# qradiolink/qradiolink

Hardware: AMD Instinct MI355X
Metric: IQ MSamples/sec through RX demod chain (higher is better)
Workload: dtype f32

## Files before the change

### qradiolink_amd/csrc/demod.hpp

```cpp
#pragma once
#include "host_common.hpp"
#include "firdes.hpp"
#include <utility>

namespace qrl {

inline std::vector<float> decim_layout(const std::vector<float>& h, int D, int Jpad)
{
    std::vector<float> t((size_t)D * Jpad, 0.0f);
    for (size_t k = 0; k < h.size(); ++k) t[(k % D) * Jpad + k / D] = h[k];
    return t;
}
inline std::vector<float> resamp_layout(const std::vector<float>& h, int I, int Jp)
{
    std::vector<float> t((size_t)I * Jp, 0.0f);
    for (size_t k = 0; k < h.size(); ++k) t[(k % I) * Jp + k / I] = h[k];
    return t;
}
inline std::vector<float2> to_f2(const std::vector<std::complex<float>>& v)
{
    std::vector<float2> r(v.size());
    for (size_t i = 0; i < v.size(); ++i) r[i] = make_float2(v[i].real(), v[i].imag());
    return r;
}

struct DecimStage {
    bool used = false;
    DecimChoice c{DECIM_CLASS_GENERIC, DECIM_R4_J12, 0};
    int D = 1, nt = 0, S = 0;
    DevBuf<float> taps;
    DevBuf<float2> edge, edge_b; uint32_t edge_len = 0;
    int alloc_edge(int B, bool two = false) {
        edge_len = (uint32_t)(c.cls == DECIM_CLASS_PM ? decim_pm_edge_len(nt, D) : c.cls == DECIM_CLASS_PL ? decim_pl_edge_len(nt, D) : 0);
        if (!edge_len) return QRL_OK;
        if (int r = edge.alloc((size_t)B * edge_len)) return r;
// ... 41 lines not shown
    DevBuf<float> f1, f2, f3; uint32_t m1 = 0, m2 = 0; DevBuf<AnState> st;
    float tone = 0.0f; DevBuf<CtcssState> cs; DevBuf<float> f4, ftaps_ct; DevBuf<double> env_ct; int nf_ct = 0;
    float wr[3] = {0, 0, 0}, wi[3] = {0, 0, 0};
    double threshold = 1e-14, ff[2] = {0, 0}, fb1 = 0, de_ff[2] = {0, 0}, de_fb1 = 0;
    float gain = 1.f, attack = 0.1f, decay = 0.1f, if_gain = 0.9f;
    int build(qrl_demod& d, size_t max2);
    int init_state(qrl_demod& d);
    int stages(qrl_demod& d, uint64_t n2_0, uint64_t n2_1, const qrl_demod_out* out, uint32_t* counts);
};

struct DsssChain {
    DevBuf<float> rs, filt, mf; int Jp = 0, nf = 0;
    DevBuf<float2> ra, rb, rc, rd, sym; uint32_t mask = 0, sym_mask = 0;
    DevBuf<DsssState> st; DevBuf<DsssTailState> tail;
    float a1 = 0, b1 = 0, a2 = 0, b2 = 0;
    uint64_t n5 = 0, nsy = 0;
    int build(qrl_demod& d, size_t max2);
    int init_state(qrl_demod& d);
    int stages(qrl_demod& d, uint64_t n2_0, uint64_t n2_1, const qrl_demod_out* out, uint32_t* counts);
};

}

using namespace qrl;

struct qrl_demod {
    qrl_ctx* ctx = nullptr;
    qrl_demod_config cfg{};
    hipStream_t stream = nullptr;
    bool own_stream = false;
    hipStream_t tail = nullptr;
    hipStream_t fecs = nullptr;
    hipEvent_t ev_q[2] = {nullptr, nullptr}, ev_fec[2] = {nullptr, nullptr}; bool q_valid[2] = {false, false};
    bool grouped = false, grouped_capable = false, fec_deferred = false; FecParams fec_pending{}; int fec_pending_slot = 0;
    DevBuf<uint64_t> qp_snap;
    hipEvent_t ev_ff = nullptr, ev_tail = nullptr;
    hipStream_t pre = nullptr; hipEvent_t ev_pre = nullptr, ev_fe[2] = {nullptr, nullptr}; bool fe_valid[2] = {false, false}; bool pre_pending = false;
    bool input_resident = false;
    hipEvent_t ev_user[4] = {nullptr, nullptr, nullptr, nullptr};
    bool tail_pending = false;
    bool qpsk_fll = false, fsk4_disc = false;
    bool m17 = false;
    DevBuf<float2> s2g, disc4_taps; DevBuf<float> sym4_taps; int disc4_nt = 0, sym4_nt = 0;
    bool fll_slim = false;
    bool d2f_capable = false, d2f = false; DevBuf<float> d2f_taps;
    bool overlap = false, overlap_capable = false; hipEvent_t ev_tail2[2] = {nullptr, nullptr}; bool tail2_valid[2] = {false, false}; uint64_t call_no = 0;
    enum Family { F_2FSK, F_GMSK, F_QPSK, F_DMR, F_4FSK, F_BPSK, F_DSSS, F_ANALOG } fam = F_2FSK;
    int branches = 2;

    int fe_decim = 1, interp = 1, decim = 1, target = 0, sps_eff = 0;
    bool fm = false;

    DecimStage fe;
    DecimStage first;
    DecimStage scope; DevBuf<float2> s_scope; uint32_t scope_mask = 0; uint64_t n_scope = 0; int scope_D = 10;
    float2* scope_out = nullptr; size_t scope_cap = 0; uint32_t* scope_counts = nullptr;
    DevBuf<float> rs_taps; int rs_Jp = 0;
    DevBuf<float> filt_taps; int filt_nt = 0;
    DevBuf<float> symf_taps; int symf_nt = 0;
    DevBuf<float2> disc_up, disc_lo; int disc_nt = 0;
    DevBuf<float> ff_tf, ff_ts; DevBuf<float2> ff_up, ff_lo;
    DevBuf<float2> fll_lo, fll_up; float fll_alpha = 0, fll_beta = 0, fll_maxf = 0;
    DevBuf<float> atan_tab, mmse_tab;
    float demod_gain = 0;
    float ss_alpha = 0, ss_beta = 0, ss_maxp = 0, ss_minp = 0;

    Rotator rot;

    DevBuf<float2> hist_a, hist_b; uint32_t hist_len = 0; bool hist_flip = false;
    DevBuf<float2> s1, s2, s2l, s2f; DevBuf<float> s2d, s3; DevBuf<uint8_t> soft;
    uint32_t s1_mask = 0, s2_mask = 0, soft_mask = 0;
    DevBuf<FllState> fll_st; DevBuf<SymSyncState> ss_st; DevBuf<FecState> fec_st;
    DevBuf<DmoState> dmo_st; DevBuf<uint32_t> dmo_golay; uint8_t* dmo_out = nullptr; uint32_t dmo_cap = 0; uint32_t* dmo_counts = nullptr;
    DevBuf<QpskState> qp_st; DevBuf<float> tanh_tab;
    float c1_alpha = 0, c1_beta = 0, c2_alpha = 0, c2_beta = 0; float2 qp_rot{};
    DevBuf<uint32_t> counts_scratch;
    AnalogChain an;
    DsssChain ds;
    uint64_t n_in = 0, n1 = 0, n2 = 0;
    bool profiling = false;
    std::vector<std::pair<hipEvent_t, hipEvent_t>> prof_events;

    ~qrl_demod() {
        for (auto& e : prof_events) { (void)hipEventDestroy(e.first); (void)hipEventDestroy(e.second); }
        if (ev_ff) (void)hipEventDestroy(ev_ff);
        if (ev_tail) (void)hipEventDestroy(ev_tail);
        for (auto e : ev_user) if (e) (void)hipEventDestroy(e);
        for (auto e : ev_tail2) if (e) (void)hipEventDestroy(e);
        for (auto e : ev_q) if (e) (void)hipEventDestroy(e);
        for (auto e : ev_fec) if (e) (void)hipEventDestroy(e);
        if (ev_pre) (void)hipEventDestroy(ev_pre);
        for (auto e : ev_fe) if (e) (void)hipEventDestroy(e);
        if (pre) (void)hipStreamDestroy(pre);
        if (fecs) (void)hipStreamDestroy(fecs);
        if (tail) (void)hipStreamDestroy(tail);
        if (own_stream && stream) (void)hipStreamDestroy(stream);
    }

    int flush_fec(bool behind_front_end);
    int sync_all() {
        if (int r = flush_fec(false)) return r;
        HIPCHK(hipStreamSynchronize(stream));
        HIPCHK(hipStreamSynchronize(tail));
        HIPCHK(hipStreamSynchronize(fecs));
        if (pre) HIPCHK(hipStreamSynchronize(pre));
        return QRL_OK;
    }
    bool loops_family() const { return fam == F_QPSK || fam == F_BPSK || fsk4_disc; }
    int init_state();
    int build();
    int process(const void* iq, size_t stride, size_t n, const qrl_demod_out* out, int fmt = IN_CF32);
    float sc16_scale = 1.0f / 32768.0f;
    int init_dmo_state() { DmoState x; std::memset(&x, 0, sizeof x); x.endPtr = 9999; return dmo_st.fill(cfg.batch, x); }
    CallCounts call_counts(size_t n) const {
        const size_t c1 = fe.used ? n / fe_decim + 2 : n, c2 = c1 * interp / decim + 2;
        return {c1, c2, c2 / (size_t)(sps_eff > 1 ? sps_eff - 1 : 1) + 8};
    }
    PortC filtered_port(const qrl_demod_out* out) const { return cfg.enable_side_outputs && out ? PortC{reinterpret_cast<float2*>(out->filtered), out->filtered_cap} : PortC{nullptr, 0}; }
    PortC constellation_port(const qrl_demod_out* out) const { return cfg.enable_side_outputs && out ? PortC{reinterpret_cast<float2*>(out->constellation), out->constellation_cap} : PortC{nullptr, 0}; }
    template <class P> void input_source(P& p, const float2* in, size_t stride, const float2* hist_old, uint64_t src0, uint64_t src1) const {
        if (fe.used) { p.in = nullptr; p.in_ring = RingC{s1.p, s1_mask}; }
        else { p.in = in; p.in_stride = stride; p.hist = hist_old; p.hist_len = hist_len; p.rot_enable = 1; rot.fill(p); }
        p.n0 = src0; p.n = (uint32_t)(src1 - src0);
// ... 3 lines not shown
```

### qradiolink_amd/csrc/engine.cpp

```cpp
#include "demod.hpp"
#include <cmath>
#include <cstdlib>
#include <memory>
#include <new>

#ifndef QRL_FEC_GATE_US
#define QRL_FEC_GATE_US 30u
#endif
#ifndef QRL_DEV_SKIP
#define QRL_DEV_SKIP 0
#endif

int qrl_demod::flush_fec(bool behind_front_end)
{
    if (!fec_deferred) return QRL_OK;
    fec_deferred = false;
    HIPCHK(hipStreamWaitEvent(fecs, ev_q[fec_pending_slot], 0));
    if (behind_front_end) {
        HIPCHK(hipStreamWaitEvent(fecs, ev_ff, 0));
        launch_fec_gate(QRL_FEC_GATE_US, fecs);
    }
    launch_fec(fec_pending, cfg.batch, fecs);
    HIPCHK(hipEventRecord(ev_fec[fec_pending_slot], fecs));
    return QRL_OK;
// ... 101 lines not shown
    const uint32_t first_look = interp == 1 ? std::max<uint32_t>(first.lookback(), d2f ? dec2_fir_lookback() : 0u) : 0u;
    {
        const int sr = cfg.time_domain_samp_rate;
        if (sr < 0 || sr > 500000 || cfg.time_domain_filter_width < 0 || cfg.time_domain_filter_width > 500000) return qrl_set_error(QRL_ERR_ARG, "time_domain_samp_rate / filter_width out of range");
        scope_D = sr > 0 ? 1000000 / sr : 10;
        if (sr > 0 && sr / 2 - sr / 8 <= 0) return qrl_set_error(QRL_ERR_ARG, "time_domain_samp_rate too small");
        const std::vector<float> h = cfg.time_domain_filter_width > 0 ? low_pass(1, 1000000, cfg.time_domain_filter_width, cfg.time_domain_filter_width, WIN_HAMMING)
                                   : sr > 0 ? low_pass(1, 1000000, sr / 2 - sr / 8, sr / 4, WIN_HAMMING)
                                            : low_pass(1, 1000000, 50000, 25000, WIN_HAMMING);
        if (h.size() > 4096) return qrl_set_error(QRL_ERR_ARG, "time-domain filter too long (> 4096 taps)");
        if ((r = scope.plan(h, scope_D))) return qrl_set_error(r, "scope plan");
    }
    if (!fe.used && (r = scope.alloc_edge(cfg.batch))) return qrl_set_error(r, "scope edge scratch");
    if (fe.used) hist_len = fe.lookback();
    else if (interp == 1) hist_len = std::max(first_look, scope.lookback());
    else hist_len = std::max((uint32_t)(rs_Jp + decim + 2), scope.lookback());
    if ((r = hist_a.alloc((size_t)B * hist_len)) || (r = hist_b.alloc((size_t)B * hist_len))) return r;

    const CallCounts mx = call_counts(cfg.max_chunk);
    if (fe.used) {
        const size_t look = std::max<size_t>(interp == 1 ? first_look : (size_t)(rs_Jp + decim + 2), scope.lookback());
        s1_mask = pow2_at_least(mx.n1 + look + 64, 64) - 1;
        if ((r = s1.alloc((size_t)B * (s1_mask + 1)))) return r;
    }
    overlap_capable = fam == F_2FSK;
    grouped_capable = fam == F_QPSK && !fsk4_disc;
    {
        int dev = 0, cus = 256; hipDeviceProp_t pr;
        if (hipGetDevice(&dev) == hipSuccess && hipGetDeviceProperties(&pr, dev) == hipSuccess) cus = pr.multiProcessorCount;
        grouped = grouped_capable && 2 * ((B + 63) / 64) >= cus;
    }
    overlap = overlap_capable;
    s2_mask = pow2_at_least((overlap_capable || loops_family() ? 2 : 1) * mx.n2 + (fam == F_DMR ? 2048 : fam == F_ANALOG ? 4096 : 1024), 64) - 1;
    const size_t ring2 = (size_t)B * (s2_mask + 1);
    if ((r = s2.alloc(ring2)) || (r = s2f.alloc(ring2)) || (r = s2d.alloc(ring2)) || (r = s3.alloc(ring2))) return r;
    if ((fam == F_2FSK || fam == F_BPSK || (fam == F_QPSK && qpsk_fll)) && (r = s2l.alloc(ring2))) return r;
    soft_mask = pow2_at_least((loops_family() ? 2 : 1) * (fam == F_QPSK || fam == F_4FSK ? 2 : 1) * mx.nsym + 512, 64) - 1;
    if ((r = soft.alloc((size_t)B * (soft_mask + 1)))) return r;

    {
        const std::vector<float> f = fam == F_QPSK
            ? root_raised_cosine(sps_eff, sps_eff, 1, 0.35, 11 * sps_eff)
            : fam == F_BPSK
            ? root_raised_cosine(sps_eff, sps_eff, 1, 0.35, 15 * sps_eff)
            : fam == F_4FSK
            ? low_pass(1, target, fw, fw / 2, WIN_BLACKMAN_HARRIS)
            : fam == F_ANALOG
            ? (an.kind == 2 ? low_pass_2(1, target, fw, 600, 90, WIN_BLACKMAN_HARRIS)
                            : low_pass_2(1, target, fw, 3500, 60, WIN_BLACKMAN_HARRIS))
            : low_pass(1, target, fw, fw, WIN_BLACKMAN_HARRIS);
        filt_nt = (int)f.size();
        if ((r = filt_taps.upload(f))) return r;
    }
    if ((r = atan_tab.upload(atan_table())) || (r = mmse_tab.upload(mmse_table()))) return r;
    if (fam == F_2FSK) {
        std::vector<std::complex<float>> lo, up;
        fll_band_edge_taps((float)sps_eff, 0.1f, 16, lo, up);
        if ((r = fll_lo.upload(to_f2(lo))) || (r = fll_up.upload(to_f2(up)))) return r;
        control_loop_gains((float)(24 * M_PI / 100), fll_alpha, fll_beta);
        fll_maxf = (float)(2 * M_PI * (2.0 / sps_eff));
        if ((r = fll_st.alloc(B))) return r;
        if (fm) {
            int nfilts = (sps == 1 ? 125 : 35) * sps_eff;
            if ((nfilts % 2) == 0) nfilts += 1;
            const std::vector<float> rrc = root_raised_cosine(1, target, target / sps_eff, 0.2, nfilts);
            symf_nt = (int)rrc.size();
// ... 83 lines not shown
            fll_maxf = (float)(2 * M_PI * (2.0 / sps_eff));
            if ((r = fll_st.alloc(B))) return r;
        }
        const float symbol_rate = (float)target / (float)sps_eff;
        const float dev = 200.0f / symbol_rate;
        clock_loop_gains((float)(2 * M_PI / (symbol_rate / 10)), 1.0f, 0.2869f, ss_alpha, ss_beta);
        ss_maxp = (float)sps_eff + dev; ss_minp = (float)sps_eff - dev;
        const float ang = (float)(-3 * M_PI / 4);
        qp_rot = make_float2((float)std::cos((double)ang), (float)std::sin((double)ang));
    } else {
        const std::vector<float> sf = low_pass(1, target, target / sps_eff, target / sps_eff, WIN_HAMMING);
        symf_nt = (int)sf.size();
        if ((r = symf_taps.upload(sf))) return r;
        demod_gain = (float)(sps_eff / (M_PI / 2));
        clock_loop_gains((float)(2 * M_PI / 200.0f), 1.0f, 0.2869f, ss_alpha, ss_beta);
        ss_maxp = (float)sps_eff + 0.05f; ss_minp = (float)sps_eff - 0.05f;
    }
    if ((r = ss_st.alloc(B)) || (r = fec_st.alloc((size_t)B * 2)) || (r = counts_scratch.alloc((size_t)B * 4))) return r;
    if (loops_family() && (r = qp_snap.alloc((size_t)B * 2))) return r;
    if ((fam == F_ANALOG && (r = an.build(*this, mx.n2))) || (fam == F_DSSS && (r = ds.build(*this, mx.n2)))) return r;
    return init_state();
}

int qrl_demod::process(const void* iq, size_t stride, size_t n, const qrl_demod_out* out, int fmt)
{
    if (fmt == IN_SC16 && !fe.used)
        return qrl_set_error(QRL_ERR_ARG, "qrl_demod_process_sc16: int16 input needs the device-rate front end (device_samp_rate >= 2000000); this handle runs at 1 Msps");
    if (n > cfg.max_chunk) return qrl_set_error(QRL_ERR_TOO_BIG, "n exceeds max_chunk");
    if (fmt == IN_SC16) {
        if (!sc16_rows_ok("qrl_demod_process_sc16", iq, stride)) return QRL_ERR_ARG;
    } else if ((reinterpret_cast<uintptr_t>(iq) & 15u) || (stride & 1u)) return qrl_set_error(QRL_ERR_ARG, "iq must be 16-byte aligned, stride even");
    const int B = cfg.batch;
    uint32_t* counts = (out && out->counts) ? out->counts : counts_scratch.p;
    hipStream_t cs = overlap ? tail : stream;
    const int slot = (int)(call_no & 1);
    if (overlap) {
        if (tail2_valid[slot]) HIPCHK(hipStreamWaitEvent(stream, ev_tail2[slot], 0));
    } else {
        HIPCHK(hipMemsetAsync(counts, 0, (size_t)B * 4 * sizeof(uint32_t), stream));
    }
    if (loops_family() && q_valid[slot]) HIPCHK(hipStreamWaitEvent(stream, ev_q[slot], 0));
    if (grouped && q_valid[slot ^ 1]) HIPCHK(hipStreamWaitEvent(stream, ev_q[slot ^ 1], 0));
    if (pre_pending) { HIPCHK(hipStreamWaitEvent(stream, ev_pre, 0)); pre_pending = false; }
    const bool use_pre = pre && input_resident;
    const float2* in = reinterpret_cast<const float2*>(iq);
    const float2* hist_old = hist_flip ? hist_b.p : hist_a.p;
    const PortC fport = filtered_port(out), cport = constellation_port(out);
    float2* hist_new = hist_flip ? hist_a.p : hist_b.p;

    const uint64_t n_in0 = n_in, n_in1 = n_in + n;
    uint64_t n1_0 = n1, n1_1 = n1;
    RingC r2{s2.p, s2_mask}, r2l{s2l.p, s2_mask}, r2f{s2f.p, s2_mask};
    RingF r2d{s2d.p, s2_mask}, r3{s3.p, s2_mask};

    hipEvent_t ev0 = nullptr, ev1 = nullptr;
    if (profiling) {
        HIPCHK(hipEventCreate(&ev0)); HIPCHK(hipEventCreate(&ev1));
        HIPCHK(hipEventRecord(ev0, stream));
    }
    if (fe.used) {
        n1_1 = decim_count(n_in1, 1, fe_decim);
        DecimParams p{};
        p.in = in; p.in_stride = stride; p.n0 = n_in0; p.n = (uint32_t)n;
        p.hist = hist_old; p.hist_len = hist_len;
        p.out = RingC{s1.p, s1_mask}; p.m0 = n1_0; p.m_count = (uint32_t)(n1_1 - n1_0);
        p.taps = fe.taps.p; p.D = fe.D; p.Jpad = fe.c.Jpad;
        p.rot_enable = 1; rot.fill(p);
        p.in_fmt = fmt; p.in_scale = sc16_scale;
        if (use_pre) { p.pre_stream = pre; p.pre_event = ev_pre; }
// ... 25 lines not shown
            p.port = fport.p; p.port_cap = fport.cap; p.port_counts = counts;
        }
        launch_resamp(p, B, stream);
    }
    if (profiling && !fe.used) { HIPCHK(hipEventRecord(ev1, stream)); prof_events.emplace_back(ev0, ev1); }
    if (scope_out) {
        const uint64_t ns_1 = decim_count(src1, 1, scope_D);
        DecimParams p{};
        input_source(p, in, stride, hist_old, src0, src1);
        p.out = RingC{s_scope.p, scope_mask}; p.m0 = n_scope; p.m_count = (uint32_t)(ns_1 - n_scope);
        p.taps = scope.taps.p; p.D = scope.D; p.Jpad = scope.c.Jpad;
        if (scope.launch(p, B, stream)) return qrl_set_error(QRL_ERR_HIP, "scope launch: hipFuncSetAttribute failed");
        launch_ring_store(RingC{s_scope.p, scope_mask}, n_scope, (uint32_t)(ns_1 - n_scope), scope_out, scope_cap, scope_counts, B, stream);
        n_scope = ns_1;
    }
    {
        HistParams h{};
        h.in = in; h.in_stride = stride; h.n0 = n_in0; h.n = (uint32_t)n;
        h.hist_old = hist_old; h.hist_new = hist_new; h.hist_len = hist_len;
        h.rot_enable = 1; rot.fill(h);
        h.in_fmt = fmt; h.in_scale = sc16_scale;
        if (pre) { HIPCHK(hipEventRecord(ev_fe[slot], stream)); fe_valid[slot] = true; }
        if (use_pre) {
            if (fe_valid[slot ^ 1]) HIPCHK(hipStreamWaitEvent(pre, ev_fe[slot ^ 1], 0));
            launch_hist_save(h, B, pre);
            HIPCHK(hipEventRecord(ev_pre, pre));
            pre_pending = true;
        } else launch_hist_save(h, B, stream);
        hist_flip = !hist_flip;
    }
    if (overlap) {
        HIPCHK(hipEventRecord(ev_ff, stream));
        HIPCHK(hipStreamWaitEvent(tail, ev_ff, 0));
        HIPCHK(hipMemsetAsync(counts, 0, (size_t)B * 4 * sizeof(uint32_t), tail));
    }
    const uint32_t c2 = (uint32_t)(n2_1 - n2_0);
    if (fam == F_DSSS || fam == F_ANALOG) {
        if (int rr = fam == F_DSSS ? ds.stages(*this, n2_0, n2_1, out, counts) : an.stages(*this, n2_0, n2_1, out, counts)) return rr;
        HIPCHK(hipGetLastError());
        if (take_launch_error()) return QRL_ERR_HIP;
        n_in = n_in1; n1 = n1_1; n2 = n2_1; ++call_no;
        return QRL_OK;
    }
    RingC filt_in = r2;
    if (fam == F_2FSK || fam == F_BPSK || (fam == F_QPSK && qpsk_fll)) {
        FllParams f{};
        f.in = r2; f.out = r2l; f.q0 = n2_0; f.count = c2; f.st = fll_st.p;
        f.lower = fll_lo.p; f.upper = fll_up.p; f.nt = fam == F_2FSK ? 16 : 32; f.alpha = fll_alpha; f.beta = fll_beta; f.max_freq = fll_maxf;
        f.slim = fll_slim ? 1 : 0;
        if (!(QRL_DEV_SKIP & 1)) launch_fll(f, B, cs);
        filt_in = r2l;
    }
    const bool fused_2fsk = fam == F_2FSK && !fm && filt_nt <= 41 && disc_nt <= 41 && symf_nt <= 25;
    if (fam == F_DMR) {
        RingC dem_in = r2;
        if (m17) {
            FirCcfParams f{};
            f.in = r2; f.out = r2f; f.q0 = n2_0; f.count = c2; f.taps = filt_taps.p; f.nt = filt_nt;
            f.port = fport.p; f.port_cap = fport.cap; f.counts = counts;
            launch_fir_ccf(f, B, cs);
            dem_in = r2f;
        }
        QuadDemodParams q{}; q.in = dem_in; q.out = r2d; q.q0 = n2_0; q.count = c2; q.gain = demod_gain; q.atan_tab = atan_tab.p;
        launch_quad_demod(q, B, cs);
        if (!overlap && tail_pending) { HIPCHK(hipStreamWaitEvent(stream, ev_tail, 0)); tail_pending = false; }
        FirFffParams f{}; f.in = r2d; f.out = r3; f.q0 = n2_0; f.count = c2; f.taps = symf_taps.p; f.nt = symf_nt;
        launch_fir_fff(f, B, cs);
        if (!overlap) { HIPCHK(hipEventRecord(ev_ff, stream)); HIPCHK(hipStreamWaitEvent(tail, ev_ff, 0)); }
    } else if (fused_2fsk) {
        if (!overlap && tail_pending) { HIPCHK(hipStreamWaitEvent(stream, ev_tail, 0)); tail_pending = false; }
        Fsk2FfParams f{};
        f.in = filt_in; f.out = r3; f.q0 = n2_0; f.count = c2;
        f.tf = ff_tf.p; f.nf = fsk2_ff_padded(filt_nt); f.up = ff_up.p; f.lo = ff_lo.p; f.nb = fsk2_ff_padded(disc_nt);
        f.ts = ff_ts.p; f.ns = fsk2_ff_padded(symf_nt);
        f.port = fport.p; f.port_cap = fport.cap; f.counts = counts;
        if (!(QRL_DEV_SKIP & 2)) launch_2fsk_ff(f, B, cs);
        if (!overlap) { HIPCHK(hipEventRecord(ev_ff, stream)); HIPCHK(hipStreamWaitEvent(tail, ev_ff, 0)); }
    } else {
        if (!d2f) {
            FirCcfParams f{};
            f.in = filt_in; f.out = r2f; f.q0 = n2_0; f.count = c2; f.taps = filt_taps.p; f.nt = filt_nt;
            f.port = fport.p; f.port_cap = fport.cap; f.counts = counts;
            launch_fir_ccf(f, B, cs);
        }
        if (fam == F_QPSK || fam == F_BPSK) {
        } else if (fsk4_disc) {
            RingC r2l4{s2l.p, s2_mask}, r2g{s2g.p, s2_mask};
            Disc4fskParams d{}; d.in = r2f; d.out = r2l4; d.q0 = n2_0; d.count = c2; d.taps = disc4_taps.p; d.nt = disc4_nt;
            launch_disc_4fsk(d, B, cs);
            FirCcfParams f{}; f.in = r2l4; f.out = r2g; f.q0 = n2_0; f.count = c2; f.taps = sym4_taps.p; f.nt = sym4_nt;
            launch_fir_ccf(f, B, cs);
        } else if (fam == F_GMSK || fam == F_4FSK || fm) {
            QuadDemodParams q{}; q.in = r2f; q.out = r2d; q.q0 = n2_0; q.count = c2; q.gain = demod_gain; q.atan_tab = atan_tab.p;
            launch_quad_demod(q, B, cs);
        } else {
            Disc2fskParams d{}; d.in = r2f; d.out = r2d; d.q0 = n2_0; d.count = c2; d.up = disc_up.p; d.lo = disc_lo.p; d.nt = disc_nt;
            launch_disc_2fsk(d, B, cs);
        }
        if (fam == F_QPSK || fam == F_BPSK || fsk4_disc) {
        } else {
            if (!overlap && tail_pending) { HIPCHK(hipStreamWaitEvent(stream, ev_tail, 0)); tail_pending = false; }
            FirFffParams f{}; f.in = r2d; f.out = r3; f.q0 = n2_0; f.count = c2; f.taps = symf_taps.p; f.nt = symf_nt;
            launch_fir_fff(f, B, cs);
            if (!overlap) { HIPCHK(hipEventRecord(ev_ff, stream)); HIPCHK(hipStreamWaitEvent(tail, ev_ff, 0)); }
        }
    }
    if (fam == F_QPSK || fam == F_BPSK || fsk4_disc) {
        QpskParams q{};
        q.in = fsk4_disc ? RingC{s2g.p, s2_mask} : r2f; q.np0 = n2_0; q.avail = n2_1; q.soft = RingB{soft.p, soft_mask}; q.st = qp_st.p;
// ... 9 lines not shown
            q.cr_omega_mid = (float)sps_eff; q.cr_omega_lim = 0.001f * (float)sps_eff;
        }
        q.port = cport.p; q.port_cap = cport.cap; q.counts = counts;
        q.oo_snap = qp_snap.p + (size_t)slot * B;
        HIPCHK(hipEventRecord(ev_ff, stream));
        HIPCHK(hipStreamWaitEvent(tail, ev_ff, 0));
        if (q_valid[slot]) HIPCHK(hipStreamWaitEvent(tail, ev_fec[slot], 0));
        launch_qpsk_loops(q, B, tail);
        HIPCHK(hipEventRecord(ev_q[slot], tail));
        if (int rf = flush_fec(true)) return rf;
        if (!grouped) HIPCHK(hipStreamWaitEvent(fecs, ev_q[slot], 0));
        FecParams f{};
        f.soft = RingB{soft.p, soft_mask};
        f.avail = q.oo_snap; f.avail_stride = sizeof(uint64_t); f.avail_mul = fam == F_BPSK ? 1 : 2;
        f.st = fec_st.p;
        f.bits_a = out ? out->bits_a : nullptr; f.bits_b = fam == F_BPSK && out ? out->bits_b : nullptr; f.bits_cap = out ? out->bits_cap : 0;
        f.counts = counts; f.branches = fam == F_BPSK ? 2 : 1;
        if (grouped) { fec_pending = f; fec_pending_slot = slot; fec_deferred = true; }
        else {
            launch_fec(f, B, fecs);
            HIPCHK(hipEventRecord(ev_fec[slot], fecs));
        }
        q_valid[slot] = true;
    } else {
        SymSyncParams s{};
        s.in = r3; s.avail = n2_1; s.soft = RingB{soft.p, soft_mask}; s.st = ss_st.p; s.mmse = mmse_tab.p;
        s.alpha = ss_alpha; s.beta = ss_beta; s.maxp = ss_maxp; s.minp = ss_minp;
        s.ted = fam == F_DMR && !m17 ? 0 : 1; s.soft_mul = 128.0f; s.soft_add = 128.0f;
        s.tail_scale = m17 ? 1.0f : 0.9f;
        s.slim = overlap ? 1 : 0;
        s.slicer = fam == F_DMR || fam == F_4FSK ? 1 : 0; s.tail = fam == F_DMR ? 1 : fam == F_4FSK ? 2 : 0;
        s.bits = out ? out->bits_a : nullptr; s.bits_cap = out ? out->bits_cap : 0;
        s.port = cport.p; s.port_cap = cport.cap; s.counts = counts;
        if (!(QRL_DEV_SKIP & 4)) launch_symsync_ff(s, B, tail);
        if (fam == F_DMR && !m17 && dmo_out) {
            DmoParams dp{}; dp.in = r3; dp.q0 = n2_0; dp.count = (uint32_t)(n2_1 - n2_0); dp.st = dmo_st.p; dp.golay = dmo_golay.p;
            dp.out = dmo_out; dp.cap = dmo_cap; dp.counts = dmo_counts;
            launch_dmo_sink(dp, B, tail);
        }
        if (fam == F_DMR) { HIPCHK(hipEventRecord(ev_tail, tail)); tail_pending = true; }
        FecParams f{};
        f.soft = RingB{soft.p, soft_mask}; f.avail = &ss_st.p[0].oo; f.avail_stride = sizeof(SymSyncState); f.avail_mul = fam == F_4FSK ? 2 : 1; f.st = fec_st.p;
        f.bits_a = out ? out->bits_a : nullptr; f.bits_b = out ? out->bits_b : nullptr; f.bits_cap = out ? out->bits_cap : 0;
        f.counts = counts; f.branches = branches;
        if (fam != F_DMR) {
            if (!(QRL_DEV_SKIP & 8)) launch_fec(f, B, tail);
            HIPCHK(hipEventRecord(ev_tail, tail));
            tail_pending = true;
        }
        if (overlap) { HIPCHK(hipEventRecord(ev_tail2[slot], tail)); tail2_valid[slot] = true; }
    }
    HIPCHK(hipGetLastError());
    if (take_launch_error()) return QRL_ERR_HIP;
    n_in = n_in1; n1 = n1_1; n2 = n2_1; ++call_no;
    return QRL_OK;
}

namespace {
struct Mode { int modem_type; qrl_demod::Family fam; int kind; bool m17, lsb; int sps, filter_width, fm; };
const Mode kModes[] = {
    {QRL_MODEM_2FSK2KFM,  qrl_demod::F_2FSK,   0, false, false, 5,   4000,   1},
    {QRL_MODEM_2FSK1KFM,  qrl_demod::F_2FSK,   0, false, false, 10,  2500,   1},
    {QRL_MODEM_2FSK2K,    qrl_demod::F_2FSK,   0, false, false, 5,   4000,   0},
    {QRL_MODEM_2FSK1K,    qrl_demod::F_2FSK,   0, false, false, 10,  2000,   0},
    {QRL_MODEM_2FSK10KFM, qrl_demod::F_2FSK,   0, false, false, 1,   25000,  1},
    {QRL_MODEM_GMSK2K,    qrl_demod::F_GMSK,   0, false, false, 5,   4000,   0},
    {QRL_MODEM_GMSK1K,    qrl_demod::F_GMSK,   0, false, false, 10,  2000,   0},
    {QRL_MODEM_GMSK10K,   qrl_demod::F_GMSK,   0, false, false, 1,   20000,  0},
    {QRL_MODEM_QPSK250K,  qrl_demod::F_QPSK,   0, false, false, 2,   160000, 0},
    {QRL_MODEM_QPSKVIDEO, qrl_demod::F_QPSK,   0, false, false, 2,   160000, 0},
    {QRL_MODEM_QPSK2K,    qrl_demod::F_QPSK,   0, false, false, 125, 1300,   0},
    {QRL_MODEM_QPSK20K,   qrl_demod::F_QPSK,   0, false, false, 25,  6500,   0},
    {QRL_MODEM_4FSK2K,    qrl_demod::F_4FSK,   0, false, false, 5,   4000,   0},
    {QRL_MODEM_4FSK2KFM,  qrl_demod::F_4FSK,   0, false, false, 5,   3000,   1},
    {QRL_MODEM_4FSK1KFM,  qrl_demod::F_4FSK,   0, false, false, 10,  2000,   1},
    {QRL_MODEM_4FSK10KFM, qrl_demod::F_4FSK,   0, false, false, 1,   20000,  1},
    {QRL_MODEM_4FSK100K,  qrl_demod::F_4FSK,   0, false, false, 2,   125000, 1},
    {QRL_MODEM_BPSK1K,    qrl_demod::F_BPSK,   0, false, false, 10,  1300,   0},
    {QRL_MODEM_BPSK2K,    qrl_demod::F_BPSK,   0, false, false, 5,   2400,   0},
    {QRL_MODEM_DMR,       qrl_demod::F_DMR,    0, false, false, 5,   5000,   0},
    {QRL_MODEM_M17,       qrl_demod::F_DMR,    0, true,  false, 125, 9000,   0},
    {QRL_MODEM_BPSK8,     qrl_demod::F_DSSS,   0, false, false, 25,  150,    0},
    {QRL_MODEM_NBFM2500,  qrl_demod::F_ANALOG, 0, false, false, 125, 2500,   0},
// ... 38 lines not shown
    for (const Mode& m : kModes) if (m.modem_type == c.modem_type) mode = &m;
    if (!mode) return qrl_set_error(QRL_ERR_ARG, "modem_type not supported by this build");
    if (c.use_mode_defaults) { c.samp_rate = 1000000; c.carrier_freq = 1700; c.sps = mode->sps; c.filter_width = mode->filter_width; c.fm = mode->fm; }
    d->fam = mode->fam; d->m17 = mode->m17; d->an.kind = mode->kind; d->an.lsb = mode->lsb;
    if (c.samp_rate != 1000000) return qrl_set_error(QRL_ERR_ARG, "internal samp_rate must be 1000000 (gr_demod_base.cpp:21)");
    if (c.device_samp_rate != 1000000 && (c.device_samp_rate < 2000000 || c.device_samp_rate % 1000000))
        return qrl_set_error(QRL_ERR_ARG, "device_samp_rate must be 1e6 or a multiple of 1e6 >= 2e6");
    HIPCHK(hipSetDevice(ctx->device));
    {
        if (c.hip_stream) d->stream = static_cast<hipStream_t>(c.hip_stream);
        else {
            int r0;
            if (std::getenv("QRL_CU_MAIN")) { if ((r0 = create_role_stream(&d->stream, 0, "MAIN"))) return r0; }
            else if (std::getenv("QRL_MAIN_PRIO_LOW")) {
                int plo = 0, phi = 0;
                (void)hipDeviceGetStreamPriorityRange(&plo, &phi);
                HIPCHK(hipStreamCreateWithPriority(&d->stream, hipStreamNonBlocking, plo));
            }
            else HIPCHK(hipStreamCreateWithFlags(&d->stream, hipStreamNonBlocking));
            d->own_stream = true;
        }
        int lo = 0, hi = 0;
        (void)hipDeviceGetStreamPriorityRange(&lo, &hi);
        int r1;
        if ((r1 = create_role_stream(&d->tail, hi, "TAIL")) || (r1 = create_role_stream(&d->fecs, lo, "FEC"))) return r1;
        if (d->own_stream && !std::getenv("QRL_NO_PRE")) { if ((r1 = create_role_stream(&d->pre, 0, "PRE"))) return r1; }
    }
    HIPCHK(hipEventCreateWithFlags(&d->ev_ff, hipEventDisableTiming));
    HIPCHK(hipEventCreateWithFlags(&d->ev_pre, hipEventDisableTiming));
    for (auto& e : d->ev_fe) HIPCHK(hipEventCreateWithFlags(&e, hipEventDisableTiming));
    HIPCHK(hipEventCreateWithFlags(&d->ev_tail, hipEventDisableTiming));
    for (auto& e : d->ev_tail2) HIPCHK(hipEventCreateWithFlags(&e, hipEventDisableTiming));
    for (auto& e : d->ev_q) HIPCHK(hipEventCreateWithFlags(&e, hipEventDisableTiming));
    for (auto& e : d->ev_fec) HIPCHK(hipEventCreateWithFlags(&e, hipEventDisableTiming));
    int r = d->build();
    if (r) return r;
    *outp = d.release();
    return QRL_OK;
}
void qrl_demod_destroy(qrl_demod* d) { if (d) { (void)d->sync_all(); delete d; } }

int qrl_demod_reset(qrl_demod* d)
{
    if (!d) return QRL_ERR_ARG;
    if (int rs = d->sync_all()) return rs;
    return d->init_state();
}
int qrl_demod_set_carrier_offset(qrl_demod* d, double hz)
{
    if (!d) return QRL_ERR_ARG;
    if (int rs = d->sync_all()) return rs;
    d->cfg.carrier_offset_hz = hz;
    return d->rot.retune(d->n_in, phase_inc_to_turn(2 * M_PI * -hz / d->cfg.device_samp_rate), d->stream);
}
int qrl_demod_set_carrier_offsets(qrl_demod* d, const double* hz)
{
    if (!d || !hz) return QRL_ERR_ARG;
    std::vector<uint64_t> ni;
    if (int r = carrier_incs(hz, d->cfg.batch, -1.0, d->cfg.device_samp_rate, ni)) return r;
    if (int rs = d->sync_all()) return rs;
    return d->rot.retune_streams(d->n_in, ni, d->stream);
}
int qrl_demod_stream_wait(qrl_demod* d, void* hip_stream)
{
    if (!d) return QRL_ERR_ARG;
    if (int rf = d->flush_fec(false)) return rf;
    hipStream_t user = static_cast<hipStream_t>(hip_stream);
    if (!d->ev_user[0]) for (auto& e : d->ev_user) HIPCHK(hipEventCreateWithFlags(&e, hipEventDisableTiming));
    HIPCHK(hipEventRecord(d->ev_user[0], d->stream));
    HIPCHK(hipEventRecord(d->ev_user[1], d->tail));
    HIPCHK(hipEventRecord(d->ev_user[2], d->fecs));
    HIPCHK(hipEventRecord(d->ev_user[3], d->pre ? d->pre : d->stream));
    for (auto e : d->ev_user) HIPCHK(hipStreamWaitEvent(user, e, 0));
    return QRL_OK;
}
int qrl_demod_set_dmo_output(qrl_demod* d, uint8_t* frames, size_t cap_frames, uint32_t* counts)
{
    if (!d) return QRL_ERR_ARG;
    if (d->fam != qrl_demod::F_DMR || d->m17) return qrl_set_error(QRL_ERR_ARG, "the DMO slicer sits behind port 3 of gr_demod_dmr: QRL_MODEM_DMR only");
    if (!frames) { if (int rs = d->sync_all()) return rs; d->dmo_out = nullptr; return QRL_OK; }
    if (!counts || cap_frames < 1 || cap_frames > 0xFFFFFFFFu) return QRL_ERR_ARG;
    int r;
    if (!d->dmo_st.p) {
        if (int rs = d->sync_all()) return rs;
        if ((r = d->dmo_st.alloc(d->cfg.batch)) || (r = d->dmo_golay.upload(golay1987_table()))) return r;
        if ((r = d->init_dmo_state())) return r;
    }
    d->dmo_out = frames; d->dmo_cap = (uint32_t)cap_frames; d->dmo_counts = counts;
    return QRL_OK;
}
int qrl_demod_set_option(qrl_demod* d, int option, int value)
{
    if (!d) return QRL_ERR_ARG;
    switch (option) {
    case QRL_OPT_OVERLAP:
        if (value != 0 && !d->overlap_capable) return qrl_set_error(QRL_ERR_ARG, "overlapped mode exists for the 2FSK family only");
        if (int rs = d->sync_all()) return rs;
        d->overlap = value != 0;
        d->tail2_valid[0] = d->tail2_valid[1] = false;
        return QRL_OK;
    case QRL_OPT_FLL_SLIM:
        if (int rs = d->sync_all()) return rs;
        d->fll_slim = value != 0;
        return QRL_OK;
    case QRL_OPT_GROUPED:
        if (value != 0 && !d->grouped_capable) return qrl_set_error(QRL_ERR_ARG, "the grouped order exists for the gr_demod_qpsk chain only");
        if (int rs = d->sync_all()) return rs;
        d->grouped = value != 0;
        return QRL_OK;
    case QRL_OPT_INPUT_RESIDENT: {
        if (int rs = d->sync_all()) return rs;
        if (value != 0 && d->pre) {
            DecimStage& st = d->fe.used ? d->fe : d->first;
            if (st.edge_len && !st.edge_b.p) if (int r = st.edge_b.alloc((size_t)d->cfg.batch * st.edge_len)) return qrl_set_error(r, "edge scratch");
        }
        d->input_resident = value != 0;
        return QRL_OK;
    }
    case QRL_OPT_UNFUSED_DEC2:
        if (!d->d2f_capable) return qrl_set_error(QRL_ERR_ARG, "this chain has no fused 1:2 decimator + shaping filter");
        if (d->n_in != 0) return qrl_set_error(QRL_ERR_STATE, "QRL_OPT_UNFUSED_DEC2 can only be set before the first sample (the two forms carry different state)");
        d->d2f = value == 0;
        return QRL_OK;
    default:
        return qrl_set_error(QRL_ERR_ARG, "unknown option");
    }
}
int qrl_demod_out_caps(const qrl_demod* d, size_t n, size_t* fcap, size_t* ccap, size_t* bcap)
{
    if (!d) return QRL_ERR_ARG;
    const CallCounts cc = d->call_counts(n);
    const size_t ns = cc.nsym;
// ... 146 lines not shown
```

### qradiolink_amd/csrc/kernels_loops.hip

```cpp
#include "devmath.hpp"
#include "engine.hpp"

namespace qrl {


#ifndef QRL_FLL_CH
#define QRL_FLL_CH 32
#endif
#ifndef QRL_FLL_TH
#define QRL_FLL_TH 256
#endif
template <int CTRL> __device__ __forceinline__ float dpp_quad(float v)
{
    return __builtin_bit_cast(float, __builtin_amdgcn_mov_dpp(__builtin_bit_cast(int, v), CTRL, 0xF, 0xF, true));
}

template <int NT, int FLL_TH, int FLL_CH>
__global__ __launch_bounds__(FLL_TH) void k_fll(const FllParams P, int batch)
{
    constexpr int FLL_NS = FLL_TH / 4;
    constexpr int GL = NT / 4;
    __shared__ float2 win[FLL_NS][FLL_CH + 1];
    __shared__ float2 tl[NT], tu[NT];
    __shared__ float2 dump[FLL_TH];
    const int tid = threadIdx.x;
    const int sl = tid >> 2, g = tid & 3;
    const int b0 = blockIdx.x * FLL_NS;
    const int b = b0 + sl;
    const bool active = b < batch;
    for (int k = tid; k < NT; k += FLL_TH) { tl[k] = P.lower[k]; tu[k] = P.upper[k]; }
    float phase = 0.f, freq = 0.f;
    float2 dl[GL];
    if (active) {
        const FllState& s = P.st[b];
// ... 50 lines not shown
                *(g == 0 ? &win[sl][k] : &dump[tid]) = y;
                dl[0] = g == 0 ? y : carry;
                {
                    const float2 v = dl[0];
                    ur = fmaf(hu[0].x, v.x, ur); ur = fmaf(-hu[0].y, v.y, ur);
                    ui = fmaf(hu[0].x, v.y, ui); ui = fmaf(hu[0].y, v.x, ui);
                    lr = fmaf(hl[0].x, v.x, lr); lr = fmaf(-hl[0].y, v.y, lr);
                    li = fmaf(hl[0].x, v.y, li); li = fmaf(hl[0].y, v.x, li);
                }
                ur = ur + dpp_quad<0xB1>(ur); ui = ui + dpp_quad<0xB1>(ui); lr = lr + dpp_quad<0xB1>(lr); li = li + dpp_quad<0xB1>(li);
                ur = ur + dpp_quad<0x4E>(ur); ui = ui + dpp_quad<0x4E>(ui); lr = lr + dpp_quad<0x4E>(lr); li = li + dpp_quad<0x4E>(li);
                const float error = (lr * lr + li * li) - (ur * ur + ui * ui);
                freq = freq + P.beta * error;
                phase = phase + freq + P.alpha * error;
                phase = phase_wrap(phase);
                freq = __builtin_fminf(__builtin_fmaxf(freq, -P.max_freq), P.max_freq);
            }
        }
        __syncthreads();
#pragma unroll
        for (int i = 0; i < NPT; ++i) {
            const int idx = tid + FLL_TH * i, s = idx / FLL_CH, k = idx % FLL_CH;
            if (s < nstreams && k < len) P.out.p[(size_t)(b0 + s) * (P.out.mask + 1u) + ((uint32_t)(P.q0 + c0 + k) & P.out.mask)] = win[s][k];
        }
    }
    if (active) {
        FllState& s = P.st[b];
        if (g == 0) { s.phase = phase; s.freq = freq; }
#pragma unroll
        for (int t = 0; t < GL; ++t) s.dl[g * GL + t] = dl[t];
    }
}

void launch_fll(const FllParams& p, int batch, hipStream_t s)
{
    if (!p.count) return;
    if (p.slim) {
        dim3 grid((batch + 15) / 16), block(64);
        if (p.nt == 16) hipLaunchKernelGGL((k_fll<16, 64, 16>), grid, block, 0, s, p, batch);
        else            hipLaunchKernelGGL((k_fll<32, 64, 16>), grid, block, 0, s, p, batch);
        return;
    }
    constexpr int TH = QRL_FLL_TH;
    dim3 grid((batch + TH / 4 - 1) / (TH / 4)), block(TH);
    if (p.nt == 16) hipLaunchKernelGGL((k_fll<16, TH, QRL_FLL_CH>), grid, block, 0, s, p, batch);
    else            hipLaunchKernelGGL((k_fll<32, TH, QRL_FLL_CH>), grid, block, 0, s, p, batch);
}

template <int NS, int W> struct SsGeo {
    static constexpr int BACK = 16;
    static constexpr int COLS = BACK + W + 8;
    static constexpr int PITCH = COLS + 1;
    static constexpr int OMAX = W == 192 ? 56 : (W + 5) * 2 / 7 + 1;
    static constexpr int OPITCH = OMAX + 1;
    static constexpr size_t lds_bytes() { return (size_t)(2 * NS * PITCH + 4 + 129 * 8 + 2 * NS * OPITCH) * sizeof(float) + 2 * 64 * sizeof(int) + (2 * 64 + 64 + 2) * sizeof(uint64_t); }
};

__device__ __forceinline__ uint64_t wave_min_u64(uint64_t v)
{
#pragma unroll
    for (int off = 32; off > 0; off >>= 1) {
        const uint64_t o = __shfl_xor((unsigned long long)v, off, 64);
        v = o < v ? o : v;
    }
    return v;
}

template <int SS_NS, int SS_W, bool VEC = false, int SS_TH = 256>
__global__ __launch_bounds__(SS_TH) void k_symsync_ff(const SymSyncParams P, int batch)
{
    using G = SsGeo<SS_NS, SS_W>;
    constexpr int SS_BACK = G::BACK, SS_COLS = G::COLS, SS_PITCH = G::PITCH, SS_OMAX = G::OMAX, SS_OPITCH = G::OPITCH;
    extern __shared__ __align__(16) unsigned char ss_smem[];
    float* win = reinterpret_cast<float*>(ss_smem);
    float* mm = win + 2 * SS_NS * SS_PITCH + 4;
    float* osym = mm + 129 * 8;
    int* ocnt = reinterpret_cast<int*>(osym + 2 * SS_NS * SS_OPITCH);
    uint64_t* obase = reinterpret_cast<uint64_t*>(ocnt + 2 * 64);
    uint64_t* oo0 = obase + 2 * 64;
// ... 233 lines not shown
```

Measured before the change: 536,300.

## Add register-window FLL kernel and split 2FSK chain into three overlapped stream stages

Adds a new FLL kernel for 16-tap band-edge filters. Each stream is handled by two lanes, which keep the delay line in registers and exchange samples with DPP quad moves instead of staging windows through LDS. For the fused 2FSK path it also moves the FLL onto the tail stream and the fused filter, symsync and FEC onto a third stream, with per-slot events, so the front end, FLL and back end of consecutive calls can run concurrently. A host-side check is added to confirm the decimated rings can hold two calls in flight. The risks are more event and stream overhead, a serial per-sample loop that exposes little parallelism, and correctness depending on the ring sizing.

```diff
diff --git a/qradiolink_amd/csrc/demod.hpp b/qradiolink_amd/csrc/demod.hpp
--- a/qradiolink_amd/csrc/demod.hpp
+++ b/qradiolink_amd/csrc/demod.hpp
@@ -1,6 +1,7 @@
 #pragma once
 #include "host_common.hpp"
 #include "firdes.hpp"
+#include "fll_plan.hpp"
 #include <utility>
 
 namespace qrl {
@@ -108,6 +109,7 @@
     hipStream_t tail = nullptr;
     hipStream_t fecs = nullptr;
     hipEvent_t ev_q[2] = {nullptr, nullptr}, ev_fec[2] = {nullptr, nullptr}; bool q_valid[2] = {false, false};
+    hipEvent_t ev_2ff[2] = {nullptr, nullptr};
     bool grouped = false, grouped_capable = false, fec_deferred = false; FecParams fec_pending{}; int fec_pending_slot = 0;
     DevBuf<uint64_t> qp_snap;
     hipEvent_t ev_ff = nullptr, ev_tail = nullptr;
@@ -165,6 +167,7 @@
         for (auto e : ev_tail2) if (e) (void)hipEventDestroy(e);
         for (auto e : ev_q) if (e) (void)hipEventDestroy(e);
         for (auto e : ev_fec) if (e) (void)hipEventDestroy(e);
+        for (auto e : ev_2ff) if (e) (void)hipEventDestroy(e);
         if (ev_pre) (void)hipEventDestroy(ev_pre);
         for (auto e : ev_fe) if (e) (void)hipEventDestroy(e);
         if (pre) (void)hipStreamDestroy(pre);
diff --git a/qradiolink_amd/csrc/engine.cpp b/qradiolink_amd/csrc/engine.cpp
--- a/qradiolink_amd/csrc/engine.cpp
+++ b/qradiolink_amd/csrc/engine.cpp
@@ -157,6 +157,10 @@
     }
     overlap = overlap_capable;
     s2_mask = pow2_at_least((overlap_capable || loops_family() ? 2 : 1) * mx.n2 + (fam == F_DMR ? 2048 : fam == F_ANALOG ? 4096 : 1024), 64) - 1;
+    if (overlap_capable) {
+        const FllStageRings rr = fll_stage_rings((uint64_t)s2_mask + 1, mx.n2, 1024, 1024);
+        if (!rr.r2_two_calls || !rr.r2l_two_calls || !rr.tail_in_order) return qrl_set_error(QRL_ERR_ARG, "decimated rings do not hold two calls");
+    }
     const size_t ring2 = (size_t)B * (s2_mask + 1);
     if ((r = s2.alloc(ring2)) || (r = s2f.alloc(ring2)) || (r = s2d.alloc(ring2)) || (r = s3.alloc(ring2))) return r;
     if ((fam == F_2FSK || fam == F_BPSK || (fam == F_QPSK && qpsk_fll)) && (r = s2l.alloc(ring2))) return r;
@@ -306,9 +310,14 @@
     } else if ((reinterpret_cast<uintptr_t>(iq) & 15u) || (stride & 1u)) return qrl_set_error(QRL_ERR_ARG, "iq must be 16-byte aligned, stride even");
     const int B = cfg.batch;
     uint32_t* counts = (out && out->counts) ? out->counts : counts_scratch.p;
-    hipStream_t cs = overlap ? tail : stream;
     const int slot = (int)(call_no & 1);
-    if (overlap) {
+    const bool fused_2fsk = fam == F_2FSK && !fm && filt_nt <= 41 && disc_nt <= 41 && symf_nt <= 25;
+    const bool fll_stage = overlap && fused_2fsk && own_stream;
+    hipStream_t ts = fll_stage ? fecs : tail;
+    hipStream_t cs = fll_stage ? ts : overlap ? tail : stream;
+    if (fll_stage) {
+        if (q_valid[slot]) HIPCHK(hipStreamWaitEvent(stream, ev_q[slot], 0));
+    } else if (overlap) {
         if (tail2_valid[slot]) HIPCHK(hipStreamWaitEvent(stream, ev_tail2[slot], 0));
     } else {
         HIPCHK(hipMemsetAsync(counts, 0, (size_t)B * 4 * sizeof(uint32_t), stream));
@@ -400,7 +409,9 @@
     if (overlap) {
         HIPCHK(hipEventRecord(ev_ff, stream));
         HIPCHK(hipStreamWaitEvent(tail, ev_ff, 0));
-        HIPCHK(hipMemsetAsync(counts, 0, (size_t)B * 4 * sizeof(uint32_t), tail));
+        if (fll_stage) {
+            if (q_valid[slot]) HIPCHK(hipStreamWaitEvent(tail, ev_2ff[slot], 0));
+        } else HIPCHK(hipMemsetAsync(counts, 0, (size_t)B * 4 * sizeof(uint32_t), tail));
     }
     const uint32_t c2 = (uint32_t)(n2_1 - n2_0);
     if (fam == F_DSSS || fam == F_ANALOG) {
@@ -416,10 +427,14 @@
         f.in = r2; f.out = r2l; f.q0 = n2_0; f.count = c2; f.st = fll_st.p;
         f.lower = fll_lo.p; f.upper = fll_up.p; f.nt = fam == F_2FSK ? 16 : 32; f.alpha = fll_alpha; f.beta = fll_beta; f.max_freq = fll_maxf;
         f.slim = fll_slim ? 1 : 0;
-        if (!(QRL_DEV_SKIP & 1)) launch_fll(f, B, cs);
+        if (!(QRL_DEV_SKIP & 1)) launch_fll(f, B, fll_stage ? tail : cs);
+        if (fll_stage) {
+            HIPCHK(hipEventRecord(ev_q[slot], tail));
+            HIPCHK(hipStreamWaitEvent(ts, ev_q[slot], 0));
+            HIPCHK(hipMemsetAsync(counts, 0, (size_t)B * 4 * sizeof(uint32_t), ts));
+        }
         filt_in = r2l;
     }
-    const bool fused_2fsk = fam == F_2FSK && !fm && filt_nt <= 41 && disc_nt <= 41 && symf_nt <= 25;
     if (fam == F_DMR) {
         RingC dem_in = r2;
         if (m17) {
@@ -443,6 +458,7 @@
         f.ts = ff_ts.p; f.ns = fsk2_ff_padded(symf_nt);
         f.port = fport.p; f.port_cap = fport.cap; f.counts = counts;
         if (!(QRL_DEV_SKIP & 2)) launch_2fsk_ff(f, B, cs);
+        if (fll_stage) { HIPCHK(hipEventRecord(ev_2ff[slot], ts)); q_valid[slot] = true; }
         if (!overlap) { HIPCHK(hipEventRecord(ev_ff, stream)); HIPCHK(hipStreamWaitEvent(tail, ev_ff, 0)); }
     } else {
         if (!d2f) {
@@ -518,23 +534,23 @@
         s.slicer = fam == F_DMR || fam == F_4FSK ? 1 : 0; s.tail = fam == F_DMR ? 1 : fam == F_4FSK ? 2 : 0;
         s.bits = out ? out->bits_a : nullptr; s.bits_cap = out ? out->bits_cap : 0;
         s.port = cport.p; s.port_cap = cport.cap; s.counts = counts;
-        if (!(QRL_DEV_SKIP & 4)) launch_symsync_ff(s, B, tail);
+        if (!(QRL_DEV_SKIP & 4)) launch_symsync_ff(s, B, ts);
         if (fam == F_DMR && !m17 && dmo_out) {
             DmoParams dp{}; dp.in = r3; dp.q0 = n2_0; dp.count = (uint32_t)(n2_1 - n2_0); dp.st = dmo_st.p; dp.golay = dmo_golay.p;
             dp.out = dmo_out; dp.cap = dmo_cap; dp.counts = dmo_counts;
-            launch_dmo_sink(dp, B, tail);
-        }
-        if (fam == F_DMR) { HIPCHK(hipEventRecord(ev_tail, tail)); tail_pending = true; }
+            launch_dmo_sink(dp, B, ts);
+        }
+        if (fam == F_DMR) { HIPCHK(hipEventRecord(ev_tail, ts)); tail_pending = true; }
         FecParams f{};
         f.soft = RingB{soft.p, soft_mask}; f.avail = &ss_st.p[0].oo; f.avail_stride = sizeof(SymSyncState); f.avail_mul = fam == F_4FSK ? 2 : 1; f.st = fec_st.p;
         f.bits_a = out ? out->bits_a : nullptr; f.bits_b = out ? out->bits_b : nullptr; f.bits_cap = out ? out->bits_cap : 0;
         f.counts = counts; f.branches = branches;
         if (fam != F_DMR) {
-            if (!(QRL_DEV_SKIP & 8)) launch_fec(f, B, tail);
-            HIPCHK(hipEventRecord(ev_tail, tail));
+            if (!(QRL_DEV_SKIP & 8)) launch_fec(f, B, ts);
+            HIPCHK(hipEventRecord(ev_tail, ts));
             tail_pending = true;
         }
-        if (overlap) { HIPCHK(hipEventRecord(ev_tail2[slot], tail)); tail2_valid[slot] = true; }
+        if (overlap) { HIPCHK(hipEventRecord(ev_tail2[slot], ts)); tail2_valid[slot] = true; }
     }
     HIPCHK(hipGetLastError());
     if (take_launch_error()) return QRL_ERR_HIP;
@@ -639,6 +655,7 @@
     HIPCHK(hipEventCreateWithFlags(&d->ev_tail, hipEventDisableTiming));
     for (auto& e : d->ev_tail2) HIPCHK(hipEventCreateWithFlags(&e, hipEventDisableTiming));
     for (auto& e : d->ev_q) HIPCHK(hipEventCreateWithFlags(&e, hipEventDisableTiming));
+    for (auto& e : d->ev_2ff) HIPCHK(hipEventCreateWithFlags(&e, hipEventDisableTiming));
     for (auto& e : d->ev_fec) HIPCHK(hipEventCreateWithFlags(&e, hipEventDisableTiming));
     int r = d->build();
     if (r) return r;
@@ -705,6 +722,7 @@
         if (int rs = d->sync_all()) return rs;
         d->overlap = value != 0;
         d->tail2_valid[0] = d->tail2_valid[1] = false;
+        if (d->fam == qrl_demod::F_2FSK) d->q_valid[0] = d->q_valid[1] = false;
         return QRL_OK;
     case QRL_OPT_FLL_SLIM:
         if (int rs = d->sync_all()) return rs;
diff --git a/qradiolink_amd/csrc/fll_plan.hpp b/qradiolink_amd/csrc/fll_plan.hpp
--- /dev/null
+++ b/qradiolink_amd/csrc/fll_plan.hpp
@@ -0,0 +1,34 @@
+#pragma once
+#include <cstdint>
+
+namespace qrl {
+
+constexpr int FLL_RW_W = 16;
+
+struct FllGrid {
+    uint64_t w0, w1;
+    int lo, hi;
+};
+constexpr FllGrid fll_rw_grid(uint64_t q0, uint32_t count)
+{
+    return FllGrid{q0 / FLL_RW_W, (q0 + count - 1) / FLL_RW_W, (int)(q0 % FLL_RW_W), (int)((q0 + count - 1) % FLL_RW_W) + 1};
+}
+constexpr int fll_rw_first_step(const FllGrid& g, uint64_t w) { return w == g.w0 ? g.lo : 0; }
+constexpr int fll_rw_end_step(const FllGrid& g, uint64_t w) { return w == g.w1 ? g.hi : FLL_RW_W; }
+
+constexpr uint32_t fll_rw_dl_entry(uint64_t n0, int r, int h, int NL)
+{
+    return (uint32_t)(h * NL) + (((uint32_t)n0 - 1u - (uint32_t)r) & (uint32_t)(NL - 1));
+}
+
+constexpr int fll_rw_slot_sample(int e, int r, int h, int NL) { return e - ((e - r) & (NL - 1)) - h * NL; }
+
+constexpr uint32_t FLL_RW_BACK = 2 * FLL_RW_W - 1;
+
+struct FllStageRings { bool r2_two_calls, r2l_two_calls, tail_in_order; };
+constexpr FllStageRings fll_stage_rings(uint64_t ring, uint64_t n2, uint64_t back_ff, uint64_t back_tail)
+{
+    return FllStageRings{2 * n2 + FLL_RW_BACK <= ring, 2 * n2 + back_ff <= ring, n2 + back_tail <= ring};
+}
+
+}
diff --git a/qradiolink_amd/csrc/kernels_loops.hip b/qradiolink_amd/csrc/kernels_loops.hip
--- a/qradiolink_amd/csrc/kernels_loops.hip
+++ b/qradiolink_amd/csrc/kernels_loops.hip
@@ -1,5 +1,6 @@
 #include "devmath.hpp"
 #include "engine.hpp"
+#include "fll_plan.hpp"
 
 namespace qrl {
 
@@ -116,6 +117,102 @@
     }
 }
 
+__global__ __launch_bounds__(64) void k_fll_rw(const FllParams P, int batch)
+{
+    constexpr int W = FLL_RW_W, NL = W / 2, GL = 4;
+    const int lane = threadIdx.x;
+    const int h = lane & 1;
+    const int b = blockIdx.x * 32 + (lane >> 1);
+    const bool active = b < batch;
+    const int bl = min(b, batch - 1);
+    const float2* __restrict__ irow = P.in.p + (size_t)bl * (P.in.mask + 1u);
+    float2* __restrict__ orow = P.out.p + (size_t)bl * (P.out.mask + 1u);
+    FllState& st = P.st[bl];
+    float phase = st.phase, freq = st.freq;
+    float2 hu[NL], hl[NL];
+#pragma unroll
+    for (int j = 0; j < NL; ++j) { hu[j] = P.upper[h * NL + j]; hl[j] = P.lower[h * NL + j]; }
+    float2 sl[NL];
+#pragma unroll
+    for (int r = 0; r < NL; ++r) sl[r] = st.dl[fll_rw_dl_entry(P.q0, r, h, NL)];
+    const FllGrid g = fll_rw_grid(P.q0, P.count);
+    float2 xc[NL];
+    {
+        const float4* q = reinterpret_cast<const float4*>(irow + (((uint32_t)(g.w0 - 1) * (uint32_t)W) & P.in.mask) + h * NL);
+#pragma unroll
+        for (int i = 0; i < NL / 2; ++i) {
+            const float4 v = q[i];
+            xc[2 * i] = g.w0 ? make_float2(v.x, v.y) : make_float2(0.f, 0.f);
+            xc[2 * i + 1] = g.w0 ? make_float2(v.z, v.w) : make_float2(0.f, 0.f);
+        }
+    }
+    for (uint64_t w = g.w0; w <= g.w1; ++w) {
+        const int lo = fll_rw_first_step(g, w), hi = fll_rw_end_step(g, w);
+        const float4* qn = reinterpret_cast<const float4*>(irow + (((uint32_t)w * (uint32_t)W) & P.in.mask) + h * NL);
+#pragma unroll
+        for (int k = 0; k < W; ++k) {
+            constexpr int M = NL - 1;
+            if (k >= lo && k < hi) {
+                float2 x;
+                if (k < NL) { x.x = dpp_quad<0xA0>(xc[k & M].x); x.y = dpp_quad<0xA0>(xc[k & M].y); }
+                else        { x.x = dpp_quad<0xF5>(xc[k & M].x); x.y = dpp_quad<0xF5>(xc[k & M].y); }
+                const float2 nco = sincos_rad(phase);
+                const float2 y = cmul(x, nco);
+                float2 carry;
+                carry.x = dpp_quad<0xB1>(sl[k & M].x);
+                carry.y = dpp_quad<0xB1>(sl[k & M].y);
+                sl[k & M] = h == 0 ? y : carry;
+                float pur[2], pui[2], plr[2], pli[2];
+#pragma unroll
+                for (int gg = 0; gg < 2; ++gg) {
+                    float ur = 0.f, ui = 0.f, lr = 0.f, li = 0.f;
+#pragma unroll
+                    for (int t = GL - 1; t >= 0; --t) {
+                        const int j = gg * GL + t;
+                        const float2 v = sl[(k - j) & M];
+                        ur = fmaf(hu[j].x, v.x, ur); ur = fmaf(-hu[j].y, v.y, ur);
+                        ui = fmaf(hu[j].x, v.y, ui); ui = fmaf(hu[j].y, v.x, ui);
+                        lr = fmaf(hl[j].x, v.x, lr); lr = fmaf(-hl[j].y, v.y, lr);
+                        li = fmaf(hl[j].x, v.y, li); li = fmaf(hl[j].y, v.x, li);
+                    }
+                    pur[gg] = ur; pui[gg] = ui; plr[gg] = lr; pli[gg] = li;
+                }
+                float ur = pur[0] + pur[1], ui = pui[0] + pui[1], lr = plr[0] + plr[1], li = pli[0] + pli[1];
+                ur = ur + dpp_quad<0xB1>(ur); ui = ui + dpp_quad<0xB1>(ui); lr = lr + dpp_quad<0xB1>(lr); li = li + dpp_quad<0xB1>(li);
+                const float error = (lr * lr + li * li) - (ur * ur + ui * ui);
+                freq = freq + P.beta * error;
+                phase = phase + freq + P.alpha * error;
+                phase = phase_wrap(phase);
+                freq = __builtin_fminf(__builtin_fmaxf(freq, -P.max_freq), P.max_freq);
+            }
+            if (k >= NL && ((k - NL) & 1)) {
+                const int r = k - NL;
+                const float4 v = qn[r / 2];
+                xc[r - 1] = make_float2(v.x, v.y); xc[r] = make_float2(v.z, v.w);
+            }
+        }
+        if (active) {
+            float2* o = orow + (((uint32_t)w * (uint32_t)W) & P.out.mask);
+            if (lo == 0 && hi == W) {
+                float4* o4 = reinterpret_cast<float4*>(o + (1 - h) * NL);
+#pragma unroll
+                for (int i = 0; i < NL / 2; ++i) o4[i] = make_float4(sl[2 * i].x, sl[2 * i].y, sl[2 * i + 1].x, sl[2 * i + 1].y);
+            } else {
+#pragma unroll
+                for (int r = 0; r < NL; ++r) {
+                    const int i = fll_rw_slot_sample(hi - 1, r, h, NL);
+                    if (i >= lo) o[i] = sl[r];
+                }
+            }
+        }
+    }
+    if (active) {
+        if (h == 0) { st.phase = phase; st.freq = freq; }
+#pragma unroll
+        for (int r = 0; r < NL; ++r) st.dl[fll_rw_dl_entry(P.q0 + P.count, r, h, NL)] = sl[r];
+    }
+}
+
 void launch_fll(const FllParams& p, int batch, hipStream_t s)
 {
     if (!p.count) return;
@@ -125,10 +222,13 @@
         else            hipLaunchKernelGGL((k_fll<32, 64, 16>), grid, block, 0, s, p, batch);
         return;
     }
+    if (p.nt == 16) {
+        hipLaunchKernelGGL(k_fll_rw, dim3((batch + 31) / 32), dim3(64), 0, s, p, batch);
+        return;
+    }
     constexpr int TH = QRL_FLL_TH;
     dim3 grid((batch + TH / 4 - 1) / (TH / 4)), block(TH);
-    if (p.nt == 16) hipLaunchKernelGGL((k_fll<16, TH, QRL_FLL_CH>), grid, block, 0, s, p, batch);
-    else            hipLaunchKernelGGL((k_fll<32, TH, QRL_FLL_CH>), grid, block, 0, s, p, batch);
+    hipLaunchKernelGGL((k_fll<32, TH, QRL_FLL_CH>), grid, block, 0, s, p, batch);
 }
 
 template <int NS, int W> struct SsGeo {
```

Result: no change. 540,000, median of 6 (+0.7%).
